# kamalmostafa/minimodem

Measured on AMD Instinct MI355X. Metric: audio samples/sec demodulated (whole node), 1200-baud 48 kHz f32, higher is better.
Workload: dtype f64; 1 GPU; configs[1]: Bell202 1200-baud, 48 kHz f32, batch of 1024 synthetic streams; 1024 streams x 480000 samples per GPU (BASELINE.json); streams_per_gpu=1024, total_streams=1024, input_dtype=f32, accumulate_dtype=f64

## Files before the change

include/mifsk.h:

```cpp
#ifndef MIFSK_H
#define MIFSK_H

#include <stddef.h>
#include <stdint.h>

#ifdef __cplusplus
extern "C" {
#endif

#define MIFSK_MAX_FRAME_BITS	64
#define MIFSK_ABI_VERSION	8

enum mifsk_decoder {
    MIFSK_DECODE_ASCII8	= 0,
    MIFSK_DECODE_BAUDOT	= 1,
    MIFSK_DECODE_BINARY	= 2,
    MIFSK_DECODE_CALLERID = 3,
    MIFSK_DECODE_UIC_GROUND = 4,
    MIFSK_DECODE_UIC_TRAIN = 5
};

typedef struct mifsk_modem_args {
    const char	*baudmode;
    unsigned	sample_rate;
// ... 92 lines not shown
    uint64_t	bits;
    float	confidence;
    float	amplitude;
    uint32_t	frame_start;
    uint32_t	n_positions;
} mifsk_search_result;

int mifsk_find_frame_batch( mifsk_ctx *ctx, const mifsk_rx_config *cfg,
	const float *d_samples,
	const mifsk_search *d_problems, mifsk_search_result *d_results,
	int nproblems, void *stream );


typedef struct mifsk_frame {
    uint64_t	bits;
    uint64_t	start;
    float	confidence;
    float	amplitude;
    uint32_t	flags;
    uint32_t	reserved;
} mifsk_frame;

#define MIFSK_FRAME_ACQUIRE	1u
#define MIFSK_FRAME_SYNC	2u
#define MIFSK_FRAME_REFINED	4u

typedef struct mifsk_episode {
    uint64_t	carrier_nsamples;
    uint32_t	first_frame;
    uint32_t	nframes;
    float	confidence_total;
    float	amplitude_total;
    uint32_t	end_reason;
    uint32_t	b_mark;
} mifsk_episode;

#define MIFSK_STREAM_FRAMES_TRUNCATED	1u
#define MIFSK_STREAM_EPISODES_TRUNCATED	2u
#define MIFSK_STREAM_ABORTED		4u

typedef struct mifsk_demod_io {
    const float		*d_samples;
    size_t		stream_stride;
    const uint32_t	*d_nsamples;
    uint32_t		nsamples;
    int			nstreams;
    uint8_t		*d_bytes;
    uint32_t		*d_nbytes;
    uint64_t		*d_bits;
    mifsk_frame		*d_frames;
    uint32_t		*d_nframes;
    size_t		frames_cap;
    mifsk_episode	*d_episodes;
    uint32_t		*d_nepisodes;
    size_t		episodes_cap;
    uint32_t		*d_status;
    uint64_t		*d_counters;
    int32_t		*d_carrier_band;
    uint32_t		flags;
    uint32_t		reserved;
} mifsk_demod_io;

#define MIFSK_IO_RING_EXACT	1u
#define MIFSK_IO_ENGINE_WORKGROUP 2u
#define MIFSK_IO_ENGINE_WAVE	4u

#define MIFSK_NCOUNTERS		32
#define MIFSK_CNT_ITERATIONS	0
#define MIFSK_CNT_BATCHES	1
#define MIFSK_CNT_STAGES	2
#define MIFSK_CNT_BULK_FRAMES	3
#define MIFSK_CNT_REFINES	4
#define MIFSK_CNT_CACHE_HITS	5
#define MIFSK_CNT_POSITIONS	6
#define MIFSK_CNT_LATTICE_BATCHES 7
#define MIFSK_CNT_CYC_TOTAL	8
#define MIFSK_CNT_CYC_PARALLEL	9
#define MIFSK_CNT_CYC_WAIT	10
#define MIFSK_CNT_CYC_CONFIDENCE 11
#define MIFSK_CNT_CYC_BULK	12
#define MIFSK_CNT_CONF_FALLBACKS 24
#define MIFSK_CNT_SEG_SECOND_LOOKS 25

int mifsk_demod_batch( mifsk_ctx *ctx, const mifsk_rx_config *cfg,
	const mifsk_demod_io *io, void *stream );


typedef struct mifsk_pipeline mifsk_pipeline;
#define MIFSK_PIPELINE_MAX_DEPTH	8
#define MIFSK_PIPELINE_NO_PRODUCER	((void *)(intptr_t)-1)

typedef struct mifsk_pipeline_info {
    uint32_t	depth_requested;
    uint32_t	depth;
    uint32_t	hw_queues;
    uint32_t	output_sets;
} mifsk_pipeline_info;

#define MIFSK_WANT_BYTES	1u
#define MIFSK_WANT_BITS		2u
#define MIFSK_WANT_FRAMES	4u
#define MIFSK_WANT_EPISODES	8u

int  mifsk_pipeline_create( mifsk_pipeline **out, int device, int depth );
void mifsk_pipeline_destroy( mifsk_pipeline *p );
int  mifsk_pipeline_info_get( const mifsk_pipeline *p, mifsk_pipeline_info *info );

int  mifsk_pipeline_outputs_alloc( mifsk_pipeline *p, int nstreams, size_t frames_cap,
	size_t episodes_cap, unsigned want );
int  mifsk_pipeline_outputs_get( mifsk_pipeline *p, uint64_t ticket, mifsk_demod_io *io );

int  mifsk_pipeline_submit( mifsk_pipeline *p, const mifsk_rx_config *cfg,
	const mifsk_demod_io *io, void *after, uint64_t *ticket );
uint64_t mifsk_pipeline_next_ticket( const mifsk_pipeline *p );
int  mifsk_pipeline_wait( mifsk_pipeline *p, uint64_t ticket );
int  mifsk_pipeline_join( mifsk_pipeline *p, uint64_t ticket, void *stream );
int  mifsk_pipeline_drain( mifsk_pipeline *p );
void *mifsk_pipeline_stream( mifsk_pipeline *p, uint64_t ticket );
mifsk_ctx *mifsk_pipeline_ctx( mifsk_pipeline *p, uint64_t ticket );


typedef struct mifsk_gather mifsk_gather;
#define MIFSK_GATHER_ID_BYTES	128
#define MIFSK_GATHER_LOOPBACK	1u

typedef struct mifsk_gather_info {
    int		rank, world, device;
    uint32_t	slots;
    uint32_t	loopback;
    uint32_t	communicator;
} mifsk_gather_info;

int  mifsk_gather_unique_id( void *id  );
int  mifsk_gather_create( mifsk_gather **out, const void *id, int rank, int world, int device,
	int slots, unsigned flags );
void mifsk_gather_destroy( mifsk_gather *g );
int  mifsk_gather_info_get( const mifsk_gather *g, mifsk_gather_info *info );
int  mifsk_gather_start( mifsk_gather *g, const uint8_t *d_bytes, size_t row_pitch,
	const int32_t *d_nbytes, int nstreams, int cols, const int *rows, void *stream,
	uint64_t *ticket );
int  mifsk_gather_received( mifsk_gather *g, uint64_t ticket, int peer,
	const uint8_t **d_bytes, const int32_t **d_nbytes, int *rows, int *cols );

typedef struct mifsk_launch_info {
    char	kernel[64];
    uint32_t	engine;
    uint32_t	workgroup_size;
    uint32_t	lds_bytes_per_workgroup;
    uint32_t	workgroups_per_cu;
    uint32_t	lattice_mode;
    uint32_t	frames_per_block;
    uint32_t	compute_units;
    uint32_t	chain_groups, chain_chunks;
} mifsk_launch_info;

int mifsk_demod_plan( mifsk_ctx *ctx, const mifsk_rx_config *cfg, int nstreams,
	unsigned flags, mifsk_launch_info *out );
int mifsk_demod_plan_ex( mifsk_ctx *ctx, const mifsk_rx_config *cfg, int nstreams,
	uint32_t nsamples, unsigned flags, mifsk_launch_info *out );


typedef struct mifsk_scan_plan {
    uint32_t	valid, nseg, npass, nwin, span_hi;
    uint32_t	pass_len[2], pass_min[2];
    float	bound_c;
    uint32_t	seg_rel[128];
// ... 202 lines not shown
```

minimodem_amd/__init__.py:

```python
import contextlib
import ctypes as C
import os
import subprocess

import numpy as np

from . import _lib
from ._lib import ModemArgs, RxConfig

__all__ = ["build", "rx_config", "Context", "demod_batch", "find_frame_batch",
           "LegacyPlan", "synthesize", "FRAME_DTYPE", "EPISODE_DTYPE",
           "gather_bytes", "shard_range"]

_HERE = os.path.dirname(os.path.abspath(__file__))

FRAME_DTYPE = np.dtype([("bits", "<u8"), ("start", "<u8"), ("confidence", "<f4"),
                        ("amplitude", "<f4"), ("flags", "<u4"), ("reserved", "<u4")])
EPISODE_DTYPE = np.dtype([("carrier_nsamples", "<u8"), ("first_frame", "<u4"),
                          ("nframes", "<u4"), ("confidence_total", "<f4"),
                          ("amplitude_total", "<f4"), ("end_reason", "<u4"),
                          ("b_mark", "<u4")])
SEARCH_DTYPE = np.dtype([("sample_offset", "<u8"), ("navail", "<u4"), ("try_first", "<u4"),
                         ("try_max", "<u4"), ("try_step", "<u4"), ("search_limit", "<f4"),
                         ("use_sync_string", "<u4")])
RESULT_DTYPE = np.dtype([("bits", "<u8"), ("confidence", "<f4"), ("amplitude", "<f4"),
                         ("frame_start", "<u4"), ("n_positions", "<u4")])
assert SEARCH_DTYPE.itemsize == 32 and RESULT_DTYPE.itemsize == 24
NCOUNTERS = 32
COUNTER_NAMES = {0: "iterations", 1: "batches", 2: "stages", 3: "bulk_frames", 4: "refines",
                 5: "cache_hits", 6: "positions", 7: "lattice_batches", 8: "cyc_total",
                 9: "cyc_scan", 10: "cyc_wait", 11: "cyc_confidence", 12: "cyc_bulk", 13: "w_stage", 14: "w_correlate",
                 15: "w_barrier", 16: "cyc_general", 17: "cyc_restart", 18: "cyc_scan1", 19: "cyc_scan2", 20: "cyc_replay_scan", 21: "cyc_scan_wait",
                 24: "conf_fallbacks", 25: "seg_second_looks"}


def build(force=False):
    if force and os.path.exists(_lib.LIB_PATH):
        os.unlink(_lib.LIB_PATH)
    subprocess.run(["make", "-s", "-C", os.path.join(_HERE, "csrc")], check=True)
    return _lib.LIB_PATH


def rx_config(baudmode="1200", **opts):
    lib = _lib.load()
    a = ModemArgs()
    lib.mifsk_modem_args_default(C.byref(a))
    a.baudmode = str(baudmode).encode()
    if "sync_byte" in opts:
        a.have_sync_byte = 1
    for k, v in opts.items():
        if not hasattr(a, k):
            raise TypeError("unknown modem option %r" % k)
        setattr(a, k, v)
    cfg = RxConfig()
    rc = lib.mifsk_rx_config_init(C.byref(cfg), C.byref(a))
    if rc != 0:
        raise ValueError("mifsk_rx_config_init failed: %d" % rc)
    cfg._keepalive = a
    return cfg


class Context:

    def __init__(self, device=-1):
        self._lib = _lib.load()
        h = C.c_void_p()
        rc = self._lib.mifsk_ctx_create(C.byref(h), int(device))
        if rc != 0:
            raise RuntimeError("mifsk_ctx_create failed: %d (no gfx950 HIP device? "
                               "this package has no CPU path)" % rc)
        self.handle = h

    @property
    def device_name(self):
        return self._lib.mifsk_ctx_device_name(self.handle).decode()

    def selftest_sqrt(self, nvalues, seed=1):
        counts = (C.c_uint64 * 4)()
        rc = self._lib.mifsk_selftest_sqrt(self.handle, int(seed), int(nvalues), counts)
        if rc != 0:
            raise RuntimeError("mifsk_selftest_sqrt failed: %d" % rc)
        return tuple(int(c) for c in counts)

    def close(self):
        if self.handle:
            self._lib.mifsk_ctx_destroy(self.handle)
            self.handle = None

    def __del__(self):
        try:
            self.close()
        except Exception:
            pass


def _torch():
    import torch
    return torch


def _on(torch, stream):
    return torch.cuda.stream(stream) if stream is not None else contextlib.nullcontext()


def _stream_ptr(torch, stream):
    if stream is None:
        stream = torch.cuda.current_stream()
    return C.c_void_p(stream.cuda_stream)


def _check_nsamples(torch, nsamples, nstreams):
    if nsamples is None:
        return
    assert nsamples.is_cuda and nsamples.dtype in (torch.int32, torch.uint32), \
        "nsamples must be a CUDA int32/uint32 tensor"
    assert nsamples.dim() == 1 and nsamples.shape[0] == nstreams and nsamples.is_contiguous()
# ... 1005 lines not shown
```

minimodem_amd/csrc/mifsk_devlib.h:

```cpp
#pragma once

#include <hip/hip_runtime.h>
#include <cfloat>
#include <cmath>
#include <cstdint>

#include "mifsk_device.h"
#include "mifsk_devmath.h"

namespace mifsk {

constexpr int P_CAP = 64;
constexpr int W_CAP = 448;


template <typename Args>
struct KernArgs {
    typedef __attribute__((address_space(4))) const Args *ptr;
    static __device__ __forceinline__ ptr here()
    {
	ptr p = (ptr)__builtin_amdgcn_kernarg_segment_ptr();
	asm volatile("" : "+s"(p));
	return p;
    }
// ... 652 lines not shown
    if ( !totals ) {
#define MIFSK_TRACK_STEP(ST, DT)										\
	"v_add_f32_dpp %[tmp], " ST ", %[av] wave_shr:1 row_mask:0xf bank_mask:0xf\n\t"		\
	"v_mul_f32_e32 " DT ", 0.5, %[tmp]\n\t"								\
	"s_nop 1\n\t"
	asm volatile(
	    "s_nop 1\n\t"
	    "s_cmp_eq_u32 %[n], 0\n\t"
	    "s_cbranch_scc1 2f\n\t"
	    "1:\n\t"
	    MIFSK_TRACK_STEP("%[xt]", "%[yt]")
	    "s_sub_u32 %[n], %[n], 1\n\t"
	    MIFSK_TRACK_STEP("%[yt]", "%[xt]")
	    "s_cmp_lg_u32 %[n], 0\n\t"
	    "s_cbranch_scc1 1b\n\t"
	    "2:\n\t"
	    "v_mov_b32_dpp %[bt], %[xt] wave_shr:1 row_mask:0xf bank_mask:0xf\n\t"
	    "s_nop 1\n\t"
	    : [bt] "+v"(bt), [xt] "+v"(xt), [yt] "+v"(yt), [tmp] "+v"(tmp), [n] "+s"(n)
	    : [av] "v"(av)
	    : "scc");
#undef MIFSK_TRACK_STEP
	return;
    }
#define MIFSK_TRACK_STEP_T(ST, SSC, SSA, DT, DSC, DSA)							\
	"v_add_f32_dpp %[tmp], " ST ", %[av] wave_shr:1 row_mask:0xf bank_mask:0xf\n\t"		\
	"v_add_f32_dpp " DSC ", " SSC ", %[cv] wave_shr:1 row_mask:0xf bank_mask:0xf\n\t"		\
	"v_mul_f32_e32 " DT ", 0.5, %[tmp]\n\t"								\
	"v_add_f32_dpp " DSA ", " SSA ", %[av] wave_shr:1 row_mask:0xf bank_mask:0xf\n\t"		\
	"s_nop 1\n\t"
    asm volatile(
	"s_nop 1\n\t"
	"s_cmp_eq_u32 %[n], 0\n\t"
	"s_cbranch_scc1 2f\n\t"
	"1:\n\t"
	MIFSK_TRACK_STEP_T("%[xt]", "%[xsc]", "%[xsa]", "%[yt]", "%[ysc]", "%[ysa]")
	"s_sub_u32 %[n], %[n], 1\n\t"
	MIFSK_TRACK_STEP_T("%[yt]", "%[ysc]", "%[ysa]", "%[xt]", "%[xsc]", "%[xsa]")
	"s_cmp_lg_u32 %[n], 0\n\t"
	"s_cbranch_scc1 1b\n\t"
	"2:\n\t"
	"v_mov_b32_dpp %[bt], %[xt] wave_shr:1 row_mask:0xf bank_mask:0xf\n\t"
	"v_mov_b32_dpp %[bsc], %[xsc] wave_shr:1 row_mask:0xf bank_mask:0xf\n\t"
	"v_mov_b32_dpp %[bsa], %[xsa] wave_shr:1 row_mask:0xf bank_mask:0xf\n\t"
	"s_nop 1\n\t"
	: [bt] "+v"(bt), [bsc] "+v"(bsc), [bsa] "+v"(bsa), [xt] "+v"(xt), [xsc] "+v"(xsc), [xsa] "+v"(xsa),
	  [yt] "+v"(yt), [ysc] "+v"(ysc), [ysa] "+v"(ysa), [tmp] "+v"(tmp), [n] "+s"(n)
	: [cv] "v"(cv), [av] "v"(av)
	: "scc");
#undef MIFSK_TRACK_STEP_T
}

__device__ __forceinline__ float wave_max_f32( float v )
{
    const float ninf = -INFINITY;
#define MIFSK_MAX_DPP(CTRL, RM)											\
    v = fmaxf(v, __builtin_bit_cast(float, __builtin_amdgcn_update_dpp(__builtin_bit_cast(int, ninf),			\
		__builtin_bit_cast(int, v), (CTRL), (RM), 0xf, false)))
    MIFSK_MAX_DPP(0x111, 0xf);
    MIFSK_MAX_DPP(0x112, 0xf);
    MIFSK_MAX_DPP(0x114, 0xf);
    MIFSK_MAX_DPP(0x118, 0xf);
    MIFSK_MAX_DPP(0x142, 0xa);
    MIFSK_MAX_DPP(0x143, 0xc);
#undef MIFSK_MAX_DPP
    return __builtin_bit_cast(float, __builtin_amdgcn_readlane(__builtin_bit_cast(int, v), 63));
}

__device__ __forceinline__ float lane_bcast( float v, uint32_t src )
{
    return __builtin_bit_cast(float,
	    __builtin_amdgcn_readlane(__builtin_bit_cast(int, v), (int)src));
}

typedef float float4_u __attribute__((ext_vector_type(4), aligned(4)));

__device__ __forceinline__ float4 load4_unaligned( const float *__restrict__ x, uint32_t a, uint32_t N )
{
    const uint32_t aa = ( a + 3 < N && a + 3 >= a ) ? a : 0u;
    const float4_u s = *reinterpret_cast<const float4_u *>(x + aa);
    return make_float4(s.x, s.y, s.z, s.w);
}


struct TwGroup {
    double	w[4];
};

typedef double double2_a16 __attribute__((ext_vector_type(2)));

__device__ __forceinline__ TwGroup tw_group_load( const double *__restrict__ tw, uint32_t g, uint32_t lane )
{
    const double *t = tw + 4 * (size_t)( 16u * g + ( lane & 15u ) );
    const double2_a16 a = *reinterpret_cast<const double2_a16 *>(t);
    const double2_a16 b = *reinterpret_cast<const double2_a16 *>(t + 2);
    TwGroup G;
    G.w[0] = a.x; G.w[1] = a.y; G.w[2] = b.x; G.w[3] = b.y;
    return G;
}

template <int J>
__device__ __forceinline__ void fmac_bcast( double &acc, const double &w, double xd )
{
    asm("v_fmac_f64_dpp %0, %1, %2 row_newbcast:%3 row_mask:0xf bank_mask:0xf"
	: "+v"(acc) : "v"(w), "v"(xd), "i"(J));
}

__device__ __forceinline__ void dpp_settle()
{
    asm volatile("s_nop 4");
}

template <int J>
__device__ __forceinline__ void fma4_bcast( double (&acc)[4], const TwGroup &G, float x )
{
    const double xd = (double)x;
    fmac_bcast<J>(acc[0], G.w[0], xd);
    fmac_bcast<J>(acc[1], G.w[1], xd);
    fmac_bcast<J>(acc[2], G.w[2], xd);
    fmac_bcast<J>(acc[3], G.w[3], xd);
}

template <int J0>
__device__ __forceinline__ void quad_bcast( double (&acc)[4], const TwGroup &G, const float4 &s )
{
    fma4_bcast<J0>(acc, G, s.x);
    fma4_bcast<J0 + 1>(acc, G, s.y);
    fma4_bcast<J0 + 2>(acc, G, s.z);
    fma4_bcast<J0 + 3>(acc, G, s.w);
}

__device__ __forceinline__ void group_bcast( double (&acc)[4], const TwGroup &G,
	const float4 &s0, const float4 &s1, const float4 &s2, const float4 &s3 )
{
    quad_bcast<0>(acc, G, s0);
    quad_bcast<4>(acc, G, s1);
    quad_bcast<8>(acc, G, s2);
    quad_bcast<12>(acc, G, s3);
}

__device__ __forceinline__ void group_bcast_tail( double (&acc)[4], const TwGroup &G,
	const float4 &s0, const float4 &s1, const float4 &s2, const float4 &s3, uint32_t cnt )
{
#define MIFSK_TAIL(J, X) if ( cnt > (J) ) fma4_bcast<J>(acc, G, X)
    MIFSK_TAIL(0, s0.x);  MIFSK_TAIL(1, s0.y);  MIFSK_TAIL(2, s0.z);   MIFSK_TAIL(3, s0.w);
    MIFSK_TAIL(4, s1.x);  MIFSK_TAIL(5, s1.y);  MIFSK_TAIL(6, s1.z);   MIFSK_TAIL(7, s1.w);
    MIFSK_TAIL(8, s2.x);  MIFSK_TAIL(9, s2.y);  MIFSK_TAIL(10, s2.z);  MIFSK_TAIL(11, s2.w);
    MIFSK_TAIL(12, s3.x); MIFSK_TAIL(13, s3.y); MIFSK_TAIL(14, s3.z);  MIFSK_TAIL(15, s3.w);
#undef MIFSK_TAIL
}

template <int NQ>
__device__ __forceinline__ void corr_lds_fixed( const TwGroup (&tg)[3], const float *p, double (&acc)[4] )
{
    static_assert(NQ >= 1 && NQ <= 12, "three resident groups");
    float4 xs[NQ];
#pragma unroll
    for ( int q = 0; q < NQ; q++ )
	xs[q] = *reinterpret_cast<const float4 *>(p + 4 * q);
    dpp_settle();
    if constexpr ( NQ == 1 ) {
	const double x0 = (double)xs[0].x;
	acc[0] = x0;
	acc[2] = x0;
	acc[1] = x0 * -0.0;
	acc[3] = acc[1];
// ... 345 lines not shown
```

minimodem_amd/csrc/mifsk_kernels.hip:

```cpp
#include <hip/hip_runtime.h>
#include <cfloat>
#include <cmath>
#include <cstdint>
#include <cstdlib>
#include <cstdio>
#include <cstring>

#include "mifsk_device.h"
#include "mifsk_devmath.h"
#include "mifsk_devlib.h"

#ifdef MIFSK_PROFILE
#define MIFSK_CLOCK() ((uint32_t)clock64())
#else
#define MIFSK_CLOCK() 0u
#endif

namespace mifsk {




__global__ __launch_bounds__(64)
void find_frame_kernel( const DevCfg *__restrict__ cfgp, const double *__restrict__ tw,
// ... 115 lines not shown
	uint32_t	anchor;
	uint32_t	frames;
	uint32_t	buf;
	uint32_t	pad;
    }		cmd[2];
    float	slab[1];
};

enum { CMD_EXIT = 0, CMD_SCAN = 1, CMD_LATTICE = 2, CMD_IDLE = 3 };




extern __shared__ __attribute__((aligned(16))) unsigned char mifsk_smem[];



__device__ __forceinline__ void par_stage( const DevCfg &cfg, StreamLds *lds, const float *__restrict__ x,
	uint32_t N, uint32_t slab_cap, uint32_t row_org, uint32_t nstage )
{
    const uint32_t org4 = row_org & ~3u;
    const uint32_t head = row_org - org4;
    const uint32_t nvec = ( nstage + head + 3 ) >> 2;
    for ( uint32_t v0 = 0; v0 < nvec; v0 += blockDim.x * STAGE_VEC ) {
	float4 buf[STAGE_VEC];
#pragma unroll
	for ( int i = 0; i < STAGE_VEC; i++ ) {
	    const uint32_t v = v0 + i * blockDim.x + threadIdx.x;
	    if ( v0 + i * blockDim.x < nvec )
		buf[i] = load4_raw(x, org4 + ( v << 2 ), N);
	}
#pragma unroll
	for ( int i = 0; i < STAGE_VEC; i++ ) {
	    const uint32_t v = v0 + i * blockDim.x + threadIdx.x;
	    if ( v0 + i * blockDim.x < nvec && v < nvec )
		store4_skewed(cfg, lds->slab, slab_cap, v << 2, head, buf[i], org4 + ( v << 2 ), N);
	}
    }
}

template <bool USE_SLAB>
__device__ __forceinline__ void par_correlate( const DevCfg &cfg, const double *__restrict__ tw, StreamLds *lds,
	const float *__restrict__ x, uint32_t N, uint32_t row_org, uint32_t nq )
{
    const uint32_t n_bits = cfg.n_bits;
    const uint32_t B = cfg.bit_nsamples;
    const uint32_t nwin = nq * n_bits;
    for ( uint32_t w0 = 0; w0 < nwin; w0 += blockDim.x ) {
	const uint32_t w = w0 + threadIdx.x;
	if ( w0 + ( threadIdx.x & ~63u ) >= nwin )
	    continue;
	const bool active = w < nwin;
	const uint32_t q = active ? udiv_magic(w, n_bits, cfg.nbits_magic) : 0;
	const uint32_t k = active ? w - q * n_bits : 0;
	const uint32_t a = lds->c_pos[q] + cfg.bit_offset[k];
	double acc[4] = { 0.0, 0.0, 0.0, 0.0 };
	if ( USE_SLAB ) {
	    corr_skewed_stream(cfg, tw, lds->slab, a - row_org, threadIdx.x & 63u, acc);
	} else {
	    for ( uint32_t n = 0; n < B; n++ ) {
		const uint32_t idx = a + n;
		const float xv = ( idx < N && idx >= a ) ? x[idx] : 0.0f;
		const double xd = (double)xv;
		const double *t = tw + 4 * (size_t)n;
		acc[0] = fma(xd, t[0], acc[0]);
		acc[1] = fma(xd, t[1], acc[1]);
		acc[2] = fma(xd, t[2], acc[2]);
		acc[3] = fma(xd, t[3], acc[3]);
	    }
	}
	if ( active )
	    lds->mags[0][w] = band_mag2(acc[0], acc[1], acc[2], acc[3], cfg.magscalar);
    }
}

template <bool USE_SLAB>
__device__ __forceinline__ void scan_part( const DevCfg &cfg, const double *__restrict__ tw,
	StreamLds *lds, const StreamLds::Cmd *cmd, const float *__restrict__ x, uint32_t N,
	uint32_t slab_cap )
{
    const uint32_t nq = cmd->nq;
    const uint32_t row_org = cmd->row_org;
    if ( USE_SLAB && cmd->stage ) {
	par_stage(cfg, lds, x, N, slab_cap, row_org, cmd->stage);
	lds_barrier();
    }
    par_correlate<USE_SLAB>(cfg, tw, lds, x, N, row_org, nq);
    lds_barrier();
}

__device__ __forceinline__ void lds_barrier()
{
    __builtin_amdgcn_fence(__ATOMIC_RELEASE, "workgroup", "local");
    __builtin_amdgcn_s_barrier();
    __builtin_amdgcn_fence(__ATOMIC_ACQUIRE, "workgroup", "local");
}



template <bool USE_SLAB>
struct Master {
    const DevCfg	&cfg;
    const double	*tw;
    const float		*x;
    uint32_t		N;
    StreamLds		*lds;
    uint32_t		slab_cap;
    uint32_t		slab_lo, slab_hi;
    uint32_t		lat_batch;
    uint32_t		conf_idx;
    uint32_t		lat_first;
    uint32_t		spec, run, cold, pause;
    uint32_t		spec_floor;
    uint32_t		lane;
    bool		inflight;
    uint32_t		inflight_anchor, inflight_frames, inflight_buf;
    uint32_t		seq;
    uint32_t		lat_n, lat_anchor;
    uint32_t		hit_base = 0xFFFFFFFFu;
    bool		cnt_on = false;
    uint32_t		cyc_par = 0, cyc_conf = 0, cyc_wait = 0, cyc_scan_wait = 0;
    uint32_t		cyc_sf_load = 0, cyc_sf_corr = 0, cyc_sf_score = 0, cyc_sf_sel = 0;
    uint32_t		h_la, h_la_magic, h_nbits;
    uint64_t		h_req_mask, h_req_val;
    TwGroup		mtg[3];

    template <int NG>
    __device__ __forceinline__ void keep_groups()
    {
#pragma unroll
	for ( int gi = 0; gi < NG; gi++ )
	    mtg[gi] = tw_group_load(tw, (uint32_t)gi, lane);
    }

    __device__ __forceinline__ Master( const DevCfg &c, const double *t, const float *xs,
	    uint32_t n, StreamLds *l, uint32_t cap, uint32_t lf, uint32_t lat_round )
	: cfg(c), tw(t), x(xs), N(n), lds(l), slab_cap(cap), slab_lo(0), slab_hi(0),
	  lat_batch(lf), lane(threadIdx.x), inflight(false), inflight_anchor(0),
	  inflight_frames(0), inflight_buf(0), seq(0), lat_n(0), lat_anchor(0)
    {
	lat_first = lat_round;
	spec = lat_batch;
	run = cold = pause = 0;
	spec_floor = 2;
	h_la = keep_scalar(cfg.lock_advance);
	h_la_magic = keep_scalar(cfg.la_magic);
	h_nbits = keep_scalar(cfg.n_bits);
	h_req_mask = keep_scalar(cfg.req_mask[0]);
	h_req_val = keep_scalar(cfg.req_val[0]);
	conf_idx = lane * cfg.n_bits;
	if ( cfg.lat_grid && lat_round ) {
	    const uint32_t r = lane / lat_round, fr = lane - r * lat_round;
	    conf_idx = r * ( lat_round * ( cfg.n_bits - 1u ) + 1u ) + fr * ( cfg.n_bits - 1u );
	}
    }

    __device__ __forceinline__ void bump( uint32_t which, uint32_t by = 1u ) const
    {
	if ( cnt_on && lane == 0 )
	    (void)__hip_atomic_fetch_add(&lds->cnt[which], by, __ATOMIC_RELAXED, __HIP_MEMORY_SCOPE_WAVEFRONT);
    }

    __device__ __forceinline__ uint32_t lattice_lookup( uint32_t p ) const
    {
	if ( !lat_n || p < lat_anchor )
	    return ~0u;
// ... 784 lines not shown
	    mifsk_stream_state st;
	    st.base = origin + base;
	    st.rp = origin + rp;
	    st.carrier_nsamples = carrier_nsamples;
	    st.nframes_total = (uint64_t)frame_base + n_out_frames;
	    st.advance = advance;
	    st.flags = MIFSK_STATE_STARTED | ( carrier ? MIFSK_STATE_CARRIER : 0u )
		     | ( paused ? 0u : MIFSK_STATE_FINISHED );
	    st.confidence_total = confidence_total;
	    st.amplitude_total = amplitude_total;
	    st.nframes_decoded = nframes_decoded;
	    st.noconfidence = noconfidence;
	    st.track_amplitude = track_amplitude;
	    st.peak_confidence = peak_confidence;
	    const bool was_started = ( rs.d_state[s].flags & MIFSK_STATE_STARTED ) != 0u;
	    st.carrier_band = was_started ? rs.d_state[s].carrier_band : -1;
	    st.first_band = was_started ? rs.d_state[s].first_band : -1;
	    st.b_mark = cfg.b_mark;
	    st.ep_b_mark = ep_b_mark;
	    st.ep_first = ep_first;
	    const uint32_t b0 = rs.append ? 0u : rs.d_state[s].nbytes_total, e0 = rs.append ? 0u : rs.d_state[s].nepisodes_total;
	    st.nbytes_total = b0 + n_out_bytes;
	    st.nepisodes_total = e0 + n_out_eps;
	    st.status = rs.d_state[s].status | status;
	    rs.d_state[s] = st;
	} else if ( stateful && t0 && ( status & MIFSK_STREAM_ABORTED ) ) {
	    mifsk_stream_state st = rs.d_state[s];
	    st.flags |= MIFSK_STATE_STARTED | MIFSK_STATE_FINISHED;
	    st.status |= MIFSK_STREAM_ABORTED;
	    rs.d_state[s] = st;
	}
    }
    if ( carrier && !( ST && ( paused || !resumable ) ) ) {
	if ( t0 && o.eps && n_out_eps < o.ecap ) {
	    mifsk_episode e;
	    e.carrier_nsamples = carrier_nsamples;
	    e.first_frame = ep_first;
	    e.nframes = nframes_decoded;
	    e.confidence_total = confidence_total;
	    e.amplitude_total = amplitude_total;
	    e.end_reason = 2;
	    e.b_mark = cfg.b_mark;
	    o.eps[n_out_eps] = e;
	}
	n_out_eps++;
    }
    if ( t0 && !( ST && rs.append != 0u && !resumable && status == 0u ) ) {
	if ( n_out_frames > o.fcap && ( o.bits || o.frames || o.bytes ) )
	    status |= MIFSK_STREAM_FRAMES_TRUNCATED;
	if ( n_out_eps > o.ecap && o.eps )
	    status |= MIFSK_STREAM_EPISODES_TRUNCATED;
	const KernArgs<DemodArgs>::ptr a = KernArgs<DemodArgs>::here();
	if ( a->io.d_nframes ) a->io.d_nframes[s] = n_out_frames;
	if ( a->io.d_nbytes ) a->io.d_nbytes[s] = n_out_bytes;
	if ( a->io.d_nepisodes ) a->io.d_nepisodes[s] = n_out_eps;
	if ( a->io.d_status ) a->io.d_status[s] = status;
	if ( a->io.d_counters ) {
	    uint64_t *c = a->io.d_counters + (size_t)s * MIFSK_NCOUNTERS;
	    for ( int i = 0; i < MIFSK_NCOUNTERS; i++ )
		c[i] = lds->cnt[i];
	    c[MIFSK_CNT_CYC_TOTAL] = MIFSK_CLOCK() - t_start;
	    c[MIFSK_CNT_CYC_PARALLEL] = ctx.cyc_par;
	    c[MIFSK_CNT_CYC_WAIT] = ctx.cyc_wait;
	    c[MIFSK_CNT_CYC_CONFIDENCE] = ctx.cyc_conf;
	    c[MIFSK_CNT_CYC_BULK] = cyc_bulk;
	    c[16] = cyc_general;
	    c[17] = cyc_restart | ( (uint64_t)ctx.cyc_sf_load << 32 );
	    c[18] = cyc_s1 | ( (uint64_t)ctx.cyc_sf_corr << 32 );
	    c[19] = cyc_s2 | ( (uint64_t)ctx.cyc_sf_score << 32 );
	    c[20] = cyc_dpp;
	    c[21] = ctx.cyc_scan_wait | ( (uint64_t)ctx.cyc_sf_sel << 32 );
#ifdef MIFSK_PROFILE
	    c[23] = ( wall_clock64() & 0xFFFFFFFFull ) | ( (uint64_t)t_wall0 << 32 );
	    c[22] = (uint64_t)( __builtin_amdgcn_s_getreg(( 3 << 11 ) | 20) & 15 ) << 32;
#endif
	}
    }
    if ( t0 )
	ctx.next_cmd()->op = CMD_EXIT;
    lds_barrier();
}


struct WorkerHot {
    uint32_t	n_bits, B, la;
    bool	grid;
    float	magscalar;
    uint32_t	buf, total, anchor0;
};

template <int NQ>
__device__ __forceinline__ void worker_lattice_linear( const WorkerHot &h, const double *__restrict__ tw,
	StreamLds *lds, const float *__restrict__ x, uint32_t N,
	uint32_t region_floats, uint32_t lat_frames, uint32_t wkr, uint32_t done, uint32_t win_base,
	uint32_t rel_lane, uint32_t safe_limit,
	float4 (&pbuf)[STAGE_VEC], uint32_t &pref_org4, uint32_t (&wcyc)[6], const TwGroup (&tgr)[3] )
{
    uint32_t lane = threadIdx.x & 63u;
    asm volatile("" : "+v"(lane));
    const uint32_t n_bits = h.n_bits, B = h.B;
    if ( h.grid )
	rel_lane = ( wkr * 64u + lane ) * B;
    const uint32_t buf = h.buf;
    float *region = lds->slab + (size_t)wkr * region_floats;
    const uint32_t total = h.total;
    {
	const uint32_t t_in = MIFSK_CLOCK();
	const uint32_t frames = total - done < lat_frames ? total - done : lat_frames;
	const uint32_t anchor = h.anchor0 + done * h.la;
	const uint32_t nwin = h.grid ? frames * ( n_bits - 1u ) + 1u : frames * n_bits;
	const uint32_t w = wkr * 64u + lane;
	if ( wkr * 64u >= nwin ) {
	    pref_org4 = 0xFFFFFFFFu;
	    return;
	}
	const bool active = w < nwin;
	const uint32_t last = nwin - wkr * 64u > 64u ? 63u : nwin - wkr * 64u - 1u;
	const uint32_t a1 = anchor + rel_lane;
	const uint32_t lo = (uint32_t)__builtin_amdgcn_readfirstlane((int)a1);
	const uint32_t hi = (uint32_t)__builtin_amdgcn_readlane((int)a1, (int)last) + B;
	const uint32_t a = active ? a1 : lo;
	const uint32_t nvec = ( hi - lo + 3 ) >> 2;

	constexpr uint32_t kRoundFloats = 64u * STAGE_VEC * 4u;
	if ( pref_org4 != lo ) {
	    const bool ok = lo <= safe_limit - kRoundFloats;
	    const float *pb = x + ( ok ? lo : 0u ) + ( lane << 2 );
#pragma unroll
	    for ( int i = 0; i < STAGE_VEC; i++ ) {
		const float4_u sv = *reinterpret_cast<const float4_u *>(pb + i * 256);
		pbuf[i] = make_float4(sv.x, sv.y, sv.z, sv.w);
	    }
	}
#ifdef MIFSK_PROFILE
	asm volatile("s_waitcnt vmcnt(0)" ::: "memory");
#endif
	const uint32_t t_a = MIFSK_CLOCK();
	float *lane_base = region + ( lane << 2 );
	const uint32_t nvec_lane = nvec > lane ? nvec - lane : 0u;
	const uint32_t elast = lo + kRoundFloats;
	if ( elast <= N && elast >= lo && region_floats >= kRoundFloats ) {
#pragma unroll
	    for ( int i = 0; i < STAGE_VEC; i++ )
		*reinterpret_cast<float4 *>(lane_base + i * 256) = pbuf[i];
	} else if ( elast <= N && elast >= lo ) {
#pragma unroll
	    for ( int i = 0; i < STAGE_VEC; i++ )
		if ( (uint32_t)( i * 64 ) < nvec_lane )
		    *reinterpret_cast<float4 *>(lane_base + i * 256) = pbuf[i];
	} else {
#pragma unroll
	    for ( int i = 0; i < STAGE_VEC; i++ ) {
		const uint32_t e = lo + ( ( i * 64 + lane ) << 2 );
		float4 sv;
		sv.x = ( e < N ) ? x[e] : 0.0f;
		sv.y = ( e + 1 < N && e + 1 > e ) ? x[e + 1] : 0.0f;
		sv.z = ( e + 2 < N && e + 2 > e ) ? x[e + 2] : 0.0f;
		sv.w = ( e + 3 < N && e + 3 > e ) ? x[e + 3] : 0.0f;
		if ( (uint32_t)( i * 64 ) < nvec_lane )
		    *reinterpret_cast<float4 *>(lane_base + i * 256) = sv;
	    }
	}
	const uint32_t t_b = MIFSK_CLOCK();
	{
	    const uint32_t nlo = lo + lat_frames * h.la;
	    const bool ok = nlo >= lo && nlo <= safe_limit - kRoundFloats;
	    const float *pb = x + ( ok ? nlo : 0u ) + ( lane << 2 );
#pragma unroll
	    for ( int i = 0; i < STAGE_VEC; i++ ) {
		const float4_u sv = *reinterpret_cast<const float4_u *>(pb + i * 256);
		pbuf[i] = make_float4(sv.x, sv.y, sv.z, sv.w);
	    }
	    pref_org4 = ok ? nlo : 0xFFFFFFFFu;
	}
	const uint32_t t_c = MIFSK_CLOCK();
	wave_lds_sync();
	const uint32_t t_mid = MIFSK_CLOCK();
	wcyc[3] += t_a - t_in;
	wcyc[4] += t_b - t_a;
	wcyc[5] += t_c - t_b;

	double mr = 0.0, mi = 0.0, sr = 0.0, si = 0.0;
	if constexpr ( NQ > 0 ) {
	    double acc[4] = { 0.0, 0.0, 0.0, 0.0 };
	    corr_lds_fixed_halves<NQ>(tgr, region + ( a - lo ), acc);
	    mr = acc[0]; mi = acc[1]; sr = acc[2]; si = acc[3];
	} else {
	    double acc[4] = { 0.0, 0.0, 0.0, 0.0 };
	    corr_lds_stream_lean(tw, region + ( a - lo ), B >> 2, lane, acc);
	    mr = acc[0]; mi = acc[1]; sr = acc[2]; si = acc[3];
	}
	if ( active )
	    lds->mags[buf][win_base + w] = band_mag2(mr, mi, sr, si, h.magscalar);
	wave_lds_sync();
	const uint32_t t_out = MIFSK_CLOCK();
	wcyc[0] += t_mid - t_in;
	wcyc[1] += t_out - t_mid;
    }
}


__device__ __forceinline__ void worker_lattice_direct( const DevCfg &cfg, const double *__restrict__ tw,
	StreamLds *lds, const StreamLds::Cmd *cmd, const float *__restrict__ x, uint32_t N,
	uint32_t lat_frames, uint32_t wkr, uint32_t done, uint32_t win_base, uint32_t (&wcyc)[6] )
{
    const uint32_t t_in = MIFSK_CLOCK();
    const uint32_t lane = threadIdx.x & 63u;
    const uint32_t n_bits = cfg.n_bits, B = cfg.bit_nsamples;
    const uint32_t total = cmd->frames;
    const uint32_t frames = total - done < lat_frames ? total - done : lat_frames;
    const uint32_t anchor = cmd->anchor + done * cfg.lock_advance;
    const uint32_t nwin = cfg.lat_grid ? frames * ( n_bits - 1u ) + 1u : frames * n_bits;
    const uint32_t w = wkr * 64u + lane;
    if ( wkr * 64u >= nwin )
	return;
    const bool active = w < nwin;
    const uint32_t wc = active ? w : wkr * 64u;
    uint32_t a;
    if ( cfg.lat_grid ) {
	a = anchor + wc * B;
    } else {
	const uint32_t f = udiv_magic(wc, n_bits, cfg.nbits_magic);
	a = anchor + f * cfg.lock_advance + cfg.bit_offset[( wc - f * n_bits ) & 63u];
    }
    const uint32_t Bpad = ( B + 15u ) & ~15u;
    double acc[4] = { 0.0, 0.0, 0.0, 0.0 };
    if ( __all(a + Bpad <= N && a + Bpad >= a) ) {
	corr_global_stream(tw, x + a, B, lane, acc);
    } else {
	for ( uint32_t n = 0; n < B; n++ ) {
	    const uint32_t idx = a + n;
	    const double xd = (double)( ( idx < N && idx >= a ) ? x[idx] : 0.0f );
	    const double *t = tw + 4 * (size_t)n;
	    acc[0] = fma(xd, t[0], acc[0]);
	    acc[1] = fma(xd, t[1], acc[1]);
	    acc[2] = fma(xd, t[2], acc[2]);
	    acc[3] = fma(xd, t[3], acc[3]);
	}
    }
    if ( active )
	lds->mags[cmd->buf][win_base + w] = band_mag2(acc[0], acc[1], acc[2], acc[3], cfg.magscalar);
    wcyc[1] += MIFSK_CLOCK() - t_in;
}

template <bool USE_SLAB, int NQ>
__device__ __forceinline__ void worker_main( const DevCfg *__restrict__ cfgp,
	const double *__restrict__ tw, StreamLds *lds, const float *__restrict__ x, uint32_t N,
	uint32_t slab_cap, uint32_t lat_frames, uint32_t region_floats, uint32_t region_cap,
	uint32_t lat_mode, uint32_t safe_limit, uint64_t *counters )
{
    const DevCfg &cfg = *cfgp;
    const uint32_t wkr = ( threadIdx.x >> 6 ) - 1u;
    uint32_t rel_lane = 0;
    if ( USE_SLAB && lat_mode == LAT_LINEAR ) {
	const uint32_t w = wkr * 64u + ( threadIdx.x & 63u );
	const uint32_t f = udiv_magic(w, cfg.n_bits, cfg.nbits_magic);
	rel_lane = cfg.lat_grid ? w * cfg.bit_nsamples
				: f * cfg.lock_advance + cfg.bit_offset[( w - f * cfg.n_bits ) & 63u];
    }
    const uint32_t wins_per_round = cfg.lat_grid ? lat_frames * ( cfg.n_bits - 1u ) + 1u
						 : lat_frames * cfg.n_bits;
    float4 pbuf[STAGE_VEC];
#pragma unroll
    for ( int i = 0; i < STAGE_VEC; i++ )
	pbuf[i] = make_float4(0.0f, 0.0f, 0.0f, 0.0f);
    TwGroup tgr[3];
    if constexpr ( NQ > 0 ) {
#pragma unroll
	for ( int gi = 0; gi < ( NQ + 3 ) / 4; gi++ )
	    tgr[gi] = tw_group_load(tw, (uint32_t)gi, threadIdx.x & 63u);
    }
    uint32_t pref_org4 = 0xFFFFFFFFu;
    uint32_t wcyc[6] = { 0, 0, 0, 0, 0, 0 };
    WorkerHot hot;
    hot.n_bits = keep_scalar(cfg.n_bits);
    hot.B = keep_scalar(cfg.bit_nsamples);
    hot.la = keep_scalar(cfg.lock_advance);
    hot.grid = cfg.lat_grid != 0u;
    hot.magscalar = keep_scalar(cfg.magscalar);
    hot.buf = hot.total = hot.anchor0 = 0u;
    for ( uint32_t seq = 0; ; seq++ ) {
	const uint32_t t_b = MIFSK_CLOCK();
	lds_barrier();
	wcyc[2] += MIFSK_CLOCK() - t_b;
	const StreamLds::Cmd *cmd = &lds->cmd[seq & 1u];
	const uint32_t op = cmd->op;
	if ( op == CMD_EXIT )
	    break;
	if ( op == CMD_SCAN ) {
	    scan_part<USE_SLAB>(cfg, tw, lds, cmd, x, N, slab_cap);
	    pref_org4 = 0xFFFFFFFFu;
#pragma unroll
	    for ( int i = 0; i < STAGE_VEC; i++ )
		pbuf[i] = make_float4(0.0f, 0.0f, 0.0f, 0.0f);
	} else if ( USE_SLAB && op == CMD_LATTICE ) {
	    if ( lat_mode == LAT_LINEAR ) {
		const uint32_t total = cmd->frames;
		hot.total = keep_scalar((uint32_t)__builtin_amdgcn_readfirstlane((int)total));
		hot.buf = keep_scalar((uint32_t)__builtin_amdgcn_readfirstlane((int)cmd->buf));
		hot.anchor0 = keep_scalar((uint32_t)__builtin_amdgcn_readfirstlane((int)cmd->anchor));
		uint32_t win_base = 0;
		for ( uint32_t done = 0; done < total; done += lat_frames, win_base += wins_per_round ) {
		    if ( lds_peek(&lds->abort) == seq + 1u )
			break;
		    worker_lattice_linear<NQ>(hot, tw, lds, x, N, region_floats, lat_frames,
					  wkr, done, win_base, rel_lane, safe_limit, pbuf, pref_org4, wcyc, tgr);
		}
	    } else if constexpr ( NQ == 0 ) {
		const uint32_t total = cmd->frames;
		uint32_t win_base = 0;
		for ( uint32_t done = 0; done < total; done += lat_frames, win_base += wins_per_round ) {
		    if ( lds_peek(&lds->abort) == seq + 1u )
			break;
		    worker_lattice_direct(cfg, tw, lds, cmd, x, N, lat_frames, wkr, done, win_base, wcyc);
		}
	    }
	}
    }
#ifdef MIFSK_PROFILE
    if ( threadIdx.x == 64 && counters ) {
	counters[13] = wcyc[0] | ( (uint64_t)wcyc[3] << 32 );
	counters[14] = wcyc[1] | ( (uint64_t)wcyc[4] << 32 );
	counters[15] = wcyc[2] | ( (uint64_t)wcyc[5] << 32 );
    }
#else
    (void)counters;
#endif
}

template <bool USE_SLAB, int NQ, int NW, bool ST = false>
__global__ __launch_bounds__(64 * ( NW + 1 ), 3)
void demod_kernel( const DevCfg *__restrict__ cfgp, const double *__restrict__ tw,
	mifsk_demod_io io, uint32_t slab_cap, uint32_t lat_frames, uint32_t lat_rounds,
	uint32_t region_floats, uint32_t region_cap, uint32_t lat_mode, WgResume rs )
{
    StreamLds *lds = reinterpret_cast<StreamLds *>(mifsk_smem);
    const uint32_t base0 = 0u;
    const DevCfg &cfg = *cfgp;

    if ( threadIdx.x == 0 )
	lds->abort = 0;
    if ( threadIdx.x < MIFSK_NCOUNTERS )
	lds->cnt[threadIdx.x] = 0;
    lds_barrier();

    uint32_t n_own = io.d_nsamples ? io.d_nsamples[blockIdx.x] : io.nsamples;
    if ( io.nstreams > 1 && (size_t)n_own > io.stream_stride )
	n_own = (uint32_t)io.stream_stride;
    const uint32_t n_row = n_own;
    if constexpr ( ST ) {
	if ( rs.d_state && rs.limit != 0u && rs.limit < n_own )
	    n_own = rs.limit;
    }
    const uint64_t rows_after = (uint64_t)( io.nstreams - 1 - (int)blockIdx.x ) * io.stream_stride;
    const uint32_t safe_limit = rows_after == 0 ? n_row
			      : rows_after > 0xFFFF0000ull ? 0xFFFF0000u : (uint32_t)rows_after;
    if ( lat_mode == LAT_LINEAR && safe_limit < 64u * STAGE_VEC * 4u )
	lat_frames = 0;

    if ( threadIdx.x < 64 ) {
	__builtin_amdgcn_s_setprio(3);
	master_loop<USE_SLAB, NQ, ST>(cfg, tw, io, slab_cap, lat_frames * lat_rounds, lat_frames, lat_mode, base0, lds, rs);
    } else {
	worker_main<USE_SLAB, NQ>(cfgp, tw, lds, io.d_samples + (size_t)blockIdx.x * io.stream_stride,
			      n_own, slab_cap, lat_frames, region_floats, region_cap, lat_mode, safe_limit,
			      io.d_counters ? io.d_counters + (size_t)blockIdx.x * MIFSK_NCOUNTERS : nullptr);
    }
}


__global__ __launch_bounds__(256)
void spectrum_kernel( const float *__restrict__ x, uint32_t nsamples,
	const double *__restrict__ cs, uint32_t fftsize, uint32_t nbands,
	float *__restrict__ mags )
{
    const uint32_t b = blockIdx.x * blockDim.x + threadIdx.x;
    if ( b >= nbands )
	return;
    double re = 0.0, im = 0.0;
    uint32_t k = 0;
    for ( uint32_t n = 0; n < nsamples; n++ ) {
	const double xd = (double)x[n];
	re = fma(xd, cs[2 * (size_t)k], re);
	im = fma(xd, cs[2 * (size_t)k + 1], im);
	k += b;
	if ( k >= fftsize )
	    k -= fftsize;
    }
    const float magscalar = 1.0f / ( (float)nsamples / 2.0f );
    mags[b] = band_mag(re, im, magscalar);
}


__global__ __launch_bounds__(256)
void selftest_sqrt_kernel( uint64_t seed, uint32_t per_thread, unsigned long long *out )
{
    uint64_t st = seed + 0x9E3779B97F4A7C15ull * ( (uint64_t)blockIdx.x * blockDim.x + threadIdx.x + 1u );
    auto next = [&]() -> uint64_t {
	uint64_t z = ( st += 0x9E3779B97F4A7C15ull );
	z = ( z ^ ( z >> 30 ) ) * 0xBF58476D1CE4E5B9ull;
	z = ( z ^ ( z >> 27 ) ) * 0x94D049BB133111EBull;
	return z ^ ( z >> 31 );
    };
    uint32_t bad = 0, guarded = 0, raw_bad = 0;
    for ( uint32_t i = 0; i < per_thread; i++ ) {
	const uint64_t r = next();
	double s;
	if ( i & 1u ) {
	    uint32_t fb = (uint32_t)r & 0x7FFFFFFFu;
	    if ( ( fb & 0x7F800000u ) == 0x7F800000u ) fb ^= 0x00800000u;
	    const float f = __uint_as_float(fb);
	    const float fn = __uint_as_float(fb + 1u);
	    const double mid = 0.5 * ( (double)f + (double)fn );
	    const long long off = (long long)( ( r >> 32 ) % 1201u ) - 600;
	    const double m = __longlong_as_double(__double_as_longlong(mid) + off);
	    s = m * m;
	} else {
	    uint32_t a = (uint32_t)r & 0x7FFFFFFFu, b = (uint32_t)( r >> 32 ) & 0x7FFFFFFFu;
	    const float fa = __uint_as_float(a), fbv = __uint_as_float(b);
	    s = __builtin_fma((double)fa, (double)fa, (double)fbv * (double)fbv);
	}
	bool unsafe;
	const float quick = (float)sqrt_newton1(s, unsafe);
	const float exact = (float)sqrt_sumsq(s);
	const bool differ = __float_as_uint(quick) != __float_as_uint(exact) && !( quick != quick && exact != exact );
	if ( unsafe )
	    guarded++;
	else if ( differ )
	    bad++;
	if ( differ )
	    raw_bad++;
    }
    atomicAdd(&out[0], (unsigned long long)bad);
    atomicAdd(&out[1], (unsigned long long)guarded);
    atomicAdd(&out[2], (unsigned long long)raw_bad);
    atomicAdd(&out[3], (unsigned long long)per_thread);
}

int launch_selftest_sqrt( uint64_t seed, uint32_t blocks, uint32_t per_thread, unsigned long long *d_out, void *stream )
{
    hipLaunchKernelGGL(selftest_sqrt_kernel, dim3(blocks), dim3(256), 0, (hipStream_t)stream, seed, per_thread, d_out);
    return hipGetLastError() == hipSuccess ? 0 : -5;
}


static inline int hip_rc( hipError_t e )
{
    return e == hipSuccess ? 0 : -5 ;
// ... 267 lines not shown
```

Measured before the change: 1536 billion samples/s.

## Use bounded buffer loads for worker prefetch with nontemporal steady-state hint

```diff
diff --git a/include/mifsk.h b/include/mifsk.h
--- a/include/mifsk.h
+++ b/include/mifsk.h
@@ -198,6 +198,13 @@
 #define MIFSK_CNT_CONF_FALLBACKS 24
 #define MIFSK_CNT_SEG_SECOND_LOOKS 25
 
+#define MIFSK_CNT_W_NEEDED_BYTES  26
+#define MIFSK_CNT_W_FETCHED_BYTES 27
+#define MIFSK_CNT_W_DROPPED_BYTES 28
+#define MIFSK_CNT_W_TAIL_BYTES    29
+#define MIFSK_CNT_STAGE_BYTES     30
+#define MIFSK_CNT_W_NT_ROUNDS     31
+
 int mifsk_demod_batch( mifsk_ctx *ctx, const mifsk_rx_config *cfg,
 	const mifsk_demod_io *io, void *stream );
 
diff --git a/minimodem_amd/__init__.py b/minimodem_amd/__init__.py
--- a/minimodem_amd/__init__.py
+++ b/minimodem_amd/__init__.py
@@ -31,7 +31,8 @@
                  5: "cache_hits", 6: "positions", 7: "lattice_batches", 8: "cyc_total",
                  9: "cyc_scan", 10: "cyc_wait", 11: "cyc_confidence", 12: "cyc_bulk", 13: "w_stage", 14: "w_correlate",
                  15: "w_barrier", 16: "cyc_general", 17: "cyc_restart", 18: "cyc_scan1", 19: "cyc_scan2", 20: "cyc_replay_scan", 21: "cyc_scan_wait",
-                 24: "conf_fallbacks", 25: "seg_second_looks"}
+                 24: "conf_fallbacks", 25: "seg_second_looks", 26: "w_needed_B", 27: "w_fetched_B",
+                 28: "w_dropped_B", 29: "w_tail_B", 30: "stage_B", 31: "w_nt_rounds"}
 
 
 def build(force=False):
diff --git a/minimodem_amd/csrc/mifsk_devlib.h b/minimodem_amd/csrc/mifsk_devlib.h
--- a/minimodem_amd/csrc/mifsk_devlib.h
+++ b/minimodem_amd/csrc/mifsk_devlib.h
@@ -758,6 +758,40 @@
     return make_float4(s.x, s.y, s.z, s.w);
 }
 
+#ifndef MIFSK_WORKER_LOAD_AUX
+#define MIFSK_WORKER_LOAD_AUX 2
+#endif
+#ifndef MIFSK_WORKER_NT_CALM
+#define MIFSK_WORKER_NT_CALM 4u
+#endif
+
+typedef float f32x4_t __attribute__((ext_vector_type(4)));
+__device__ f32x4_t raw_buffer_load_f32x4( __amdgpu_buffer_rsrc_t rsrc, int voffset, int soffset, int aux )
+    __asm("llvm.amdgcn.raw.ptr.buffer.load.v4f32");
+
+template <int AUX>
+__device__ __forceinline__ void round_load( float4 (&pbuf)[STAGE_VEC], const float *__restrict__ x,
+	uint32_t from, uint32_t nfloats, uint32_t lane )
+{
+    const uint64_t p = reinterpret_cast<uint64_t>(x + from);
+    const uint32_t plo = (uint32_t)__builtin_amdgcn_readfirstlane((int)(uint32_t)p);
+    const uint32_t phi = (uint32_t)__builtin_amdgcn_readfirstlane((int)(uint32_t)( p >> 32 ));
+    const uint32_t nbytes = (uint32_t)__builtin_amdgcn_readfirstlane((int)( nfloats << 2 ));
+    void *base = reinterpret_cast<void *>(( (uint64_t)phi << 32 ) | plo);
+    const __amdgpu_buffer_rsrc_t rs = __builtin_amdgcn_make_buffer_rsrc(base, (short)0, (int)nbytes, 0x00020000);
+    uint32_t off[( STAGE_VEC + 3 ) / 4];
+#pragma unroll
+    for ( int k = 0; k < ( STAGE_VEC + 3 ) / 4; k++ ) {
+	off[k] = ( lane << 4 ) + 4096u * k;
+	asm volatile("" : "+v"(off[k]));
+    }
+#pragma unroll
+    for ( int i = 0; i < STAGE_VEC; i++ ) {
+	const f32x4_t v = raw_buffer_load_f32x4(rs, (int)( off[i >> 2] + 1024u * ( i & 3 ) ), 0, AUX);
+	pbuf[i] = make_float4(v.x, v.y, v.z, v.w);
+    }
+}
+
 
 struct TwGroup {
     double	w[4];
diff --git a/minimodem_amd/csrc/mifsk_kernels.hip b/minimodem_amd/csrc/mifsk_kernels.hip
--- a/minimodem_amd/csrc/mifsk_kernels.hip
+++ b/minimodem_amd/csrc/mifsk_kernels.hip
@@ -221,6 +221,11 @@
     const uint32_t nq = cmd->nq;
     const uint32_t row_org = cmd->row_org;
     if ( USE_SLAB && cmd->stage ) {
+#ifdef MIFSK_PROFILE
+	if ( threadIdx.x == 0 )
+	    (void)__hip_atomic_fetch_add(&lds->cnt[MIFSK_CNT_STAGE_BYTES], ( ( cmd->stage + ( row_org & 3u ) + 3u ) >> 2 ) << 4,
+					 __ATOMIC_RELAXED, __HIP_MEMORY_SCOPE_WORKGROUP);
+#endif
 	par_stage(cfg, lds, x, N, slab_cap, row_org, cmd->stage);
 	lds_barrier();
     }
@@ -1171,10 +1176,21 @@
 }
 
 
+__device__ __forceinline__ void worker_bump( StreamLds *lds, uint32_t which, uint32_t by )
+{
+#ifdef MIFSK_PROFILE
+    if ( ( threadIdx.x & 63u ) == 0u )
+	(void)__hip_atomic_fetch_add(&lds->cnt[which], by, __ATOMIC_RELAXED, __HIP_MEMORY_SCOPE_WORKGROUP);
+#else
+    (void)lds; (void)which; (void)by;
+#endif
+}
+
 struct WorkerHot {
     uint32_t	n_bits, B, la;
     bool	grid;
     float	magscalar;
+    uint32_t	nvec_full;
     uint32_t	buf, total, anchor0;
 };
 
@@ -1182,8 +1198,9 @@
 __device__ __forceinline__ void worker_lattice_linear( const WorkerHot &h, const double *__restrict__ tw,
 	StreamLds *lds, const float *__restrict__ x, uint32_t N,
 	uint32_t region_floats, uint32_t lat_frames, uint32_t wkr, uint32_t done, uint32_t win_base,
-	uint32_t rel_lane, uint32_t safe_limit,
-	float4 (&pbuf)[STAGE_VEC], uint32_t &pref_org4, uint32_t (&wcyc)[6], const TwGroup (&tgr)[3] )
+	uint32_t rel_lane,
+	float4 (&pbuf)[STAGE_VEC], uint32_t &pref_org4, uint32_t &calm, uint32_t &pref_bytes,
+	uint32_t (&wcyc)[6], const TwGroup (&tgr)[3] )
 {
     uint32_t lane = threadIdx.x & 63u;
     asm volatile("" : "+v"(lane));
@@ -1200,6 +1217,8 @@
 	const uint32_t nwin = h.grid ? frames * ( n_bits - 1u ) + 1u : frames * n_bits;
 	const uint32_t w = wkr * 64u + lane;
 	if ( wkr * 64u >= nwin ) {
+	    if ( pref_org4 != 0xFFFFFFFFu )
+		worker_bump(lds, MIFSK_CNT_W_DROPPED_BYTES, pref_bytes);
 	    pref_org4 = 0xFFFFFFFFu;
 	    return;
 	}
@@ -1210,16 +1229,16 @@
 	const uint32_t hi = (uint32_t)__builtin_amdgcn_readlane((int)a1, (int)last) + B;
 	const uint32_t a = active ? a1 : lo;
 	const uint32_t nvec = ( hi - lo + 3 ) >> 2;
-
 	constexpr uint32_t kRoundFloats = 64u * STAGE_VEC * 4u;
-	if ( pref_org4 != lo ) {
-	    const bool ok = lo <= safe_limit - kRoundFloats;
-	    const float *pb = x + ( ok ? lo : 0u ) + ( lane << 2 );
-#pragma unroll
-	    for ( int i = 0; i < STAGE_VEC; i++ ) {
-		const float4_u sv = *reinterpret_cast<const float4_u *>(pb + i * 256);
-		pbuf[i] = make_float4(sv.x, sv.y, sv.z, sv.w);
-	    }
+
+	worker_bump(lds, MIFSK_CNT_W_NEEDED_BYTES, ( hi - lo ) << 2);
+	if ( pref_org4 != lo || nvec > h.nvec_full ) {
+	    const uint32_t nf = lo < N ? min(nvec << 2, N - lo) : 0u;
+	    round_load<0>(pbuf, x, lo, nf, lane);
+	    if ( pref_org4 != 0xFFFFFFFFu )
+		worker_bump(lds, MIFSK_CNT_W_DROPPED_BYTES, pref_bytes);
+	    worker_bump(lds, MIFSK_CNT_W_FETCHED_BYTES, nf << 2);
+	    calm = 0u;
 	}
 #ifdef MIFSK_PROFILE
 	asm volatile("s_waitcnt vmcnt(0)" ::: "memory");
@@ -1227,7 +1246,7 @@
 	const uint32_t t_a = MIFSK_CLOCK();
 	float *lane_base = region + ( lane << 2 );
 	const uint32_t nvec_lane = nvec > lane ? nvec - lane : 0u;
-	const uint32_t elast = lo + kRoundFloats;
+	const uint32_t elast = lo + ( nvec << 2 );
 	if ( elast <= N && elast >= lo && region_floats >= kRoundFloats ) {
 #pragma unroll
 	    for ( int i = 0; i < STAGE_VEC; i++ )
@@ -1238,6 +1257,7 @@
 		if ( (uint32_t)( i * 64 ) < nvec_lane )
 		    *reinterpret_cast<float4 *>(lane_base + i * 256) = pbuf[i];
 	} else {
+	    worker_bump(lds, MIFSK_CNT_W_TAIL_BYTES, lo < N ? min(nvec << 2, N - lo) << 2 : 0u);
 #pragma unroll
 	    for ( int i = 0; i < STAGE_VEC; i++ ) {
 		const uint32_t e = lo + ( ( i * 64 + lane ) << 2 );
@@ -1253,14 +1273,18 @@
 	const uint32_t t_b = MIFSK_CLOCK();
 	{
 	    const uint32_t nlo = lo + lat_frames * h.la;
-	    const bool ok = nlo >= lo && nlo <= safe_limit - kRoundFloats;
-	    const float *pb = x + ( ok ? nlo : 0u ) + ( lane << 2 );
-#pragma unroll
-	    for ( int i = 0; i < STAGE_VEC; i++ ) {
-		const float4_u sv = *reinterpret_cast<const float4_u *>(pb + i * 256);
-		pbuf[i] = make_float4(sv.x, sv.y, sv.z, sv.w);
-	    }
+	    const bool ok = nlo >= lo && nlo < N;
+	    const uint32_t nf = ok ? min(h.nvec_full << 2, N - nlo) : 0u;
+	    if ( calm >= MIFSK_WORKER_NT_CALM ) {
+		round_load<MIFSK_WORKER_LOAD_AUX>(pbuf, x, ok ? nlo : 0u, nf, lane);
+		worker_bump(lds, MIFSK_CNT_W_NT_ROUNDS, 1u);
+	    } else {
+		round_load<0>(pbuf, x, ok ? nlo : 0u, nf, lane);
+	    }
+	    calm++;
 	    pref_org4 = ok ? nlo : 0xFFFFFFFFu;
+	    pref_bytes = nf << 2;
+	    worker_bump(lds, MIFSK_CNT_W_FETCHED_BYTES, nf << 2);
 	}
 	const uint32_t t_c = MIFSK_CLOCK();
 	wave_lds_sync();
@@ -1336,7 +1360,7 @@
 __device__ __forceinline__ void worker_main( const DevCfg *__restrict__ cfgp,
 	const double *__restrict__ tw, StreamLds *lds, const float *__restrict__ x, uint32_t N,
 	uint32_t slab_cap, uint32_t lat_frames, uint32_t region_floats, uint32_t region_cap,
-	uint32_t lat_mode, uint32_t safe_limit, uint64_t *counters )
+	uint32_t lat_mode, uint64_t *counters )
 {
     const DevCfg &cfg = *cfgp;
     const uint32_t wkr = ( threadIdx.x >> 6 ) - 1u;
@@ -1349,6 +1373,13 @@
     }
     const uint32_t wins_per_round = cfg.lat_grid ? lat_frames * ( cfg.n_bits - 1u ) + 1u
 						 : lat_frames * cfg.n_bits;
+    uint32_t nvec_full = 0;
+    if ( USE_SLAB && lat_mode == LAT_LINEAR && wins_per_round > wkr * 64u ) {
+	const uint32_t last = wins_per_round - wkr * 64u > 64u ? 63u : wins_per_round - wkr * 64u - 1u;
+	const uint32_t r0 = (uint32_t)__builtin_amdgcn_readfirstlane((int)rel_lane);
+	const uint32_t r1 = (uint32_t)__builtin_amdgcn_readlane((int)rel_lane, (int)last) + cfg.bit_nsamples;
+	nvec_full = ( r1 - r0 + 3u ) >> 2;
+    }
     float4 pbuf[STAGE_VEC];
 #pragma unroll
     for ( int i = 0; i < STAGE_VEC; i++ )
@@ -1359,7 +1390,7 @@
 	for ( int gi = 0; gi < ( NQ + 3 ) / 4; gi++ )
 	    tgr[gi] = tw_group_load(tw, (uint32_t)gi, threadIdx.x & 63u);
     }
-    uint32_t pref_org4 = 0xFFFFFFFFu;
+    uint32_t pref_org4 = 0xFFFFFFFFu, calm = 0u, pref_bytes = 0u;
     uint32_t wcyc[6] = { 0, 0, 0, 0, 0, 0 };
     WorkerHot hot;
     hot.n_bits = keep_scalar(cfg.n_bits);
@@ -1367,6 +1398,7 @@
     hot.la = keep_scalar(cfg.lock_advance);
     hot.grid = cfg.lat_grid != 0u;
     hot.magscalar = keep_scalar(cfg.magscalar);
+    hot.nvec_full = keep_scalar((uint32_t)__builtin_amdgcn_readfirstlane((int)nvec_full));
     hot.buf = hot.total = hot.anchor0 = 0u;
     for ( uint32_t seq = 0; ; seq++ ) {
 	const uint32_t t_b = MIFSK_CLOCK();
@@ -1377,6 +1409,9 @@
 	if ( op == CMD_EXIT )
 	    break;
 	if ( op == CMD_SCAN ) {
+	    if ( pref_org4 != 0xFFFFFFFFu )
+		worker_bump(lds, MIFSK_CNT_W_DROPPED_BYTES, pref_bytes);
+	    calm = 0u;
 	    scan_part<USE_SLAB>(cfg, tw, lds, cmd, x, N, slab_cap);
 	    pref_org4 = 0xFFFFFFFFu;
 #pragma unroll
@@ -1393,7 +1428,7 @@
 		    if ( lds_peek(&lds->abort) == seq + 1u )
 			break;
 		    worker_lattice_linear<NQ>(hot, tw, lds, x, N, region_floats, lat_frames,
-					  wkr, done, win_base, rel_lane, safe_limit, pbuf, pref_org4, wcyc, tgr);
+					  wkr, done, win_base, rel_lane, pbuf, pref_org4, calm, pref_bytes, wcyc, tgr);
 		}
 	    } else if constexpr ( NQ == 0 ) {
 		const uint32_t total = cmd->frames;
@@ -1407,6 +1442,9 @@
 	}
     }
 #ifdef MIFSK_PROFILE
+    if ( ( threadIdx.x & 63u ) == 0u && counters && pref_org4 != 0xFFFFFFFFu )
+	atomicAdd(reinterpret_cast<unsigned long long *>(counters + MIFSK_CNT_W_DROPPED_BYTES),
+		  (unsigned long long)pref_bytes);
     if ( threadIdx.x == 64 && counters ) {
 	counters[13] = wcyc[0] | ( (uint64_t)wcyc[3] << 32 );
 	counters[14] = wcyc[1] | ( (uint64_t)wcyc[4] << 32 );
@@ -1436,23 +1474,17 @@
     uint32_t n_own = io.d_nsamples ? io.d_nsamples[blockIdx.x] : io.nsamples;
     if ( io.nstreams > 1 && (size_t)n_own > io.stream_stride )
 	n_own = (uint32_t)io.stream_stride;
-    const uint32_t n_row = n_own;
     if constexpr ( ST ) {
 	if ( rs.d_state && rs.limit != 0u && rs.limit < n_own )
 	    n_own = rs.limit;
     }
-    const uint64_t rows_after = (uint64_t)( io.nstreams - 1 - (int)blockIdx.x ) * io.stream_stride;
-    const uint32_t safe_limit = rows_after == 0 ? n_row
-			      : rows_after > 0xFFFF0000ull ? 0xFFFF0000u : (uint32_t)rows_after;
-    if ( lat_mode == LAT_LINEAR && safe_limit < 64u * STAGE_VEC * 4u )
-	lat_frames = 0;
 
     if ( threadIdx.x < 64 ) {
 	__builtin_amdgcn_s_setprio(3);
 	master_loop<USE_SLAB, NQ, ST>(cfg, tw, io, slab_cap, lat_frames * lat_rounds, lat_frames, lat_mode, base0, lds, rs);
     } else {
 	worker_main<USE_SLAB, NQ>(cfgp, tw, lds, io.d_samples + (size_t)blockIdx.x * io.stream_stride,
-			      n_own, slab_cap, lat_frames, region_floats, region_cap, lat_mode, safe_limit,
+			      n_own, slab_cap, lat_frames, region_floats, region_cap, lat_mode,
 			      io.d_counters ? io.d_counters + (size_t)blockIdx.x * MIFSK_NCOUNTERS : nullptr);
     }
 }
```

New measurement: 1509 billion samples/s (median of 2 runs). -1.7%, worse.
